# nmoehrle/mvs-texturing

Measured on AMD Instinct MI355X. Metric: faces/sec through view-selection (data-cost + MRF), higher is better.
Workload: dtype f32; 1 GPU; BASELINE config 3: displaced icosphere n=316 (1997120 faces), 200 Fibonacci-sphere views 2048x1536 RGB8, settings gmi/none/visibility-test (reference defaults); faces=1997120, views=200, nnz=88914367, sweeps=39, icm_iters=10, partition=library-hilbert-1, face_order_in=as built, msg_bits=8, max_labels=0

## Files before the change

### mvs-texturing_amd/csrc/ctx.h

```cpp
#pragma once
#include <hip/hip_runtime.h>
#include <stdint.h>
#include <string.h>
#include <algorithm>
#include <functional>
#include <stdexcept>
#include <string>
#include <vector>

#include "../../include/mvs_viewsel.h"
#include "dmath.h"

namespace mvs {

struct HipError : std::runtime_error {
    explicit HipError(const std::string& m) : std::runtime_error(m) {}
};
struct StatusError : std::runtime_error {
    mvs_status st;
    StatusError(mvs_status s, const std::string& m) : std::runtime_error(m), st(s) {}
};

#define MVS_HIP(expr)                                                                          \
    do {                                                                                       \
// ... 133 lines not shown
    mvs::DBuf<size_t> view_off;
    bool mesh_dirty = true, views_dirty = true;

    int face_order = 1;
    mvs::DBuf<float> i_verts, i_normals; mvs::DBuf<uint32_t> i_faces, f_perm, f_pos, f_tmp;
    const float* iv = nullptr; const uint32_t* ifc = nullptr; const float* inr = nullptr;
    bool mesh_ordered = false;
    bool order_pinned = false;
    const uint32_t* t_perm = nullptr; const uint32_t* t_pos = nullptr;
    mvs::DBuf<uint32_t> u_ptr, u_cnt; mvs::DBuf<uint16_t> u_view; mvs::DBuf<float> u_cost, u_q;
    bool u_valid = false, u_q_valid = false;
    mvs::DBuf<unsigned long long> fp_acc;
    mvs::HBuf<uint32_t> stage_ptr; mvs::HBuf<uint16_t> stage_view[2]; mvs::HBuf<float> stage_cost[2];

    mvs::DBuf<mvs::Node4> bvh_nodes; mvs::DBuf<float4> bvh_tris;
    mvs::DBuf<uint32_t> sort_k, sort_k2, sort_v, sort_v2; mvs::DBuf<char> sort_tmp;
    mvs::DBuf<float> lvl_box_a, lvl_box_b; mvs::DBuf<float> scene_box;
    mvs::BvhDev bvh{};
    mvs::DBuf<uint32_t> vf_ptr, vf_cursor, vf;
    mvs::DBuf<uint32_t> vperm, vpos;
    const uint32_t* tri_order = nullptr;

    mvs::DBuf<unsigned long long> pass_bits, need_bits, occl_bits, surv_bits;
    mvs::DBuf<uint32_t> pass_base;
    mvs::DBuf<uint32_t> pass_face;
    mvs::DBuf<unsigned long long> defer_bits; mvs::DBuf<uint32_t> defer_base; mvs::DBuf<uint2> defer_list; mvs::DBuf<uint32_t> rewalk_list;
    mvs::DBuf<float> pq;
    mvs::DBuf<float> pcol;
    mvs::DBuf<uint32_t> face_cnt, scan_tmp;
    mvs::DBuf<unsigned long long> counters;
    mvs::DBuf<float> max_q; mvs::DBuf<uint32_t> hist; mvs::DBuf<float> pctl;
    mvs::DBuf<uint32_t> pre_ptr; mvs::DBuf<uint16_t> pre_view; mvs::DBuf<float> pre_q; mvs::DBuf<float> pre_col;
    mvs::DBuf<uint8_t> pre_inl;
    mvs::DBuf<uint32_t> csr_ptr; mvs::DBuf<uint16_t> csr_view; mvs::DBuf<float> csr_cost; mvs::DBuf<float> csr_q;
    uint32_t csr_faces = 0, csr_views = 0; uint64_t csr_nnz = 0;
    const uint32_t* r_ptr = nullptr; const uint16_t* r_view = nullptr; const float* r_cost = nullptr;
    bool csr_q_valid = false;
    bool have_costs = false;
    mvs_settings dc_settings{}; mvs_dc_stats dc_stats{}; int dc_phase = 0;

    mvs::DBuf<unsigned long long> g_keys, g_keys2; mvs::DBuf<uint32_t> g_vals, g_vals2, g_pos, g_cnt, g_adj_ptr, g_adj, g_faces; mvs::DBuf<float> g_normals;
    uint64_t g_adj_entries = 0; bool have_adj = false;

    mvs::DBuf<uint32_t> p_label_ptr, p_comp_ptr, p_comp_faces, p_parent, p_root, p_state, p_flag, p_pos, p_roots, p_roots2, p_rlab, p_rlab2, p_adj_ptr, p_adj, p_labels;

    mvs::DBuf<uint32_t> row_adj_ptr, row_adj, row_labels; mvs::HBuf<char> row_pin;
// ... 93 lines not shown
```

### mvs-texturing_amd/csrc/dmath.h

```cpp
#pragma once
#include <stdint.h>
#include <math.h>
#include <float.h>
#include <string.h>

#if defined(__HIPCC__)
#define MVS_HD __host__ __device__ __forceinline__
#else
#define MVS_HD inline
#endif

namespace mvs {

struct V3 { float x, y, z; };
struct V2 { float x, y; };

MVS_HD V3 operator+(V3 a, V3 b) { return {a.x + b.x, a.y + b.y, a.z + b.z}; }
MVS_HD V3 operator-(V3 a, V3 b) { return {a.x - b.x, a.y - b.y, a.z - b.z}; }
MVS_HD V3 operator/(V3 a, float s) { return {a.x / s, a.y / s, a.z / s}; }
MVS_HD float dot(V3 a, V3 b) { return (a.x * b.x + a.y * b.y) + a.z * b.z; }
MVS_HD float norm(V3 a) { return sqrtf(dot(a, a)); }
MVS_HD V3 normalized(V3 a) { return a / norm(a); }
MVS_HD V3 cross(V3 a, V3 b) {
    return {a.y * b.z - a.z * b.y, a.z * b.x - a.x * b.z, a.x * b.y - a.y * b.x};
// ... 123 lines not shown
    float ext = 0.0f, mag = 0.0f;
    for (int a = 0; a < 3; ++a) {
        ext = fmaxf(ext, hi[a] - lo[a]);
        mag = fmaxf(mag, fmaxf(fabsf(lo[a]), fabsf(hi[a])));
    }
    return 1e-5f * fmaxf(ext, mag) + 1e-30f;
}

MVS_HD void tri_pad_box(V3 a, V3 e1, V3 e2, float pad, V3* lo, V3* hi) {
    const V3 b = a + e1, c = a + e2;
    lo->x = fminf(a.x, fminf(b.x, c.x)) - pad; hi->x = fmaxf(a.x, fmaxf(b.x, c.x)) + pad;
    lo->y = fminf(a.y, fminf(b.y, c.y)) - pad; hi->y = fmaxf(a.y, fmaxf(b.y, c.y)) + pad;
    lo->z = fminf(a.z, fminf(b.z, c.z)) - pad; hi->z = fmaxf(a.z, fmaxf(b.z, c.z)) + pad;
}
MVS_HD float dot_fma(V3 a, V3 b) { return __builtin_fmaf(a.z, b.z, __builtin_fmaf(a.y, b.y, a.x * b.x)); }
MVS_HD V3 cross_fma(V3 a, V3 b) {
    return V3{__builtin_fmaf(a.y, b.z, -(a.z * b.y)), __builtin_fmaf(a.z, b.x, -(a.x * b.z)), __builtin_fmaf(a.x, b.y, -(a.y * b.x))};
}
MVS_HD bool ray_tri_point_in_box(const Ray& r, float tn, float det, V3 lo, V3 hi) {
    const float t = tn / det;
    const float hx = r.o.x + t * r.d.x, hy = r.o.y + t * r.d.y, hz = r.o.z + t * r.d.z;
    return hx >= lo.x && hx <= hi.x && hy >= lo.y && hy <= hi.y && hz >= lo.z && hz <= hi.z;
}
MVS_HD bool ray_tri_boxed(const Ray& r, V3 a, V3 e1, V3 e2, V3 lo, V3 hi) {
    const V3 pv = cross_fma(r.d, e2);
    const float det = dot_fma(e1, pv);
    const V3 tv = r.o - a;
    const float un = dot_fma(tv, pv);
    const V3 qv = cross_fma(tv, e1);
    const float vn = dot_fma(r.d, qv);
    const float tn = dot_fma(e2, qv);
    const float sg = det < 0.0f ? -1.0f : 1.0f;
    const float ad = det * sg, us = un * sg, vs = vn * sg, ts = tn * sg;
    const float w = ad - (us + vs);
    const float g1 = __builtin_fmaf(-r.tmin, ad, ts), g2 = __builtin_fmaf(r.tmax, ad, -ts);
    const bool pre = (ad > 0.0f) & (fminf(fminf(fminf(fminf(us, vs), w), g1), g2) >= 0.0f);
    if (!pre) return false;
    return ray_tri_point_in_box(r, tn, det, lo, hi);
}
MVS_HD bool ray_tri(const Ray& r, V3 a, V3 e1, V3 e2) {
    V3 lo, hi;
    tri_pad_box(a, e1, e2, r.pad, &lo, &hi);
    return ray_tri_boxed(r, a, e1, e2, lo, hi);
}

MVS_HD uint8_t linear_at(const uint8_t* img, int w, int h, int chans, float x, float y, int c) {
    x = smax(0.0f, smin((float)(w - 1), x));
    y = smax(0.0f, smin((float)(h - 1), y));
    const int floor_x = (int)x, floor_y = (int)y;
    const int floor_xp1 = imin(floor_x + 1, w - 1), floor_yp1 = imin(floor_y + 1, h - 1);
    const float w1 = x - (float)floor_x, w0 = 1.0f - w1;
    const float w3 = y - (float)floor_y, w2 = 1.0f - w3;
    const int rowstride = w * chans;
    const size_t row1 = (size_t)floor_y * rowstride, row2 = (size_t)floor_yp1 * rowstride;
    const int col1 = floor_x * chans, col2 = floor_xp1 * chans;
    const float v1 = img[row1 + col1 + c], v2 = img[row1 + col2 + c];
    const float v3 = img[row2 + col1 + c], v4 = img[row2 + col2 + c];
    return (uint8_t)(((v1 * (w0 * w2) + v2 * (w1 * w2)) + v3 * (w0 * w3)) + v4 * (w1 * w3) + 0.5f);
}

// ... 261 lines not shown
```

### mvs-texturing_amd/csrc/k_bvh.hip

```cpp
#include "ctx.h"
#include <rocprim/rocprim.hpp>
#ifndef MVS_LEAF_T
#define MVS_LEAF_T 16
#endif

namespace mvs {

namespace {

constexpr uint32_t LEAF_T = MVS_LEAF_T;
constexpr int LEAF_SLOTS = 64 / (int)LEAF_T;

__device__ __forceinline__ uint32_t f2ord(float f) {
    uint32_t u = __float_as_uint(f);
    return (u & 0x80000000u) ? ~u : (u | 0x80000000u);
}
__device__ __forceinline__ float ord2f(uint32_t u) {
    return __uint_as_float((u & 0x80000000u) ? (u & 0x7FFFFFFFu) : ~u);
}

__global__ void __launch_bounds__(256) bbox_kernel(const float* __restrict__ verts, uint32_t n_verts, uint32_t* __restrict__ part ) {
    __shared__ uint32_t s_red[4][6];
    float lo[3] = {INFINITY, INFINITY, INFINITY}, hi[3] = {-INFINITY, -INFINITY, -INFINITY};
    for (uint32_t v = blockIdx.x * blockDim.x + threadIdx.x; v < n_verts; v += gridDim.x * blockDim.x)
// ... 156 lines not shown
    float lo[3], hi[3];
    for (int a = 0; a < 3; ++a) { lo[a] = ord2f(box[a]); hi[a] = ord2f(box[3 + a]); }
    return scene_pad(lo, hi);
}

constexpr uint32_t TRI_F4 = 4;
__global__ void gather_tris_kernel(const float* __restrict__ verts, const uint32_t* __restrict__ faces, const uint32_t* __restrict__ order,
                                   uint32_t n_faces, uint32_t n_slots, const uint32_t* __restrict__ scene_box, float4* __restrict__ tris) {
    const uint32_t s = blockIdx.x * blockDim.x + threadIdx.x;
    if (s >= n_slots) return;
    float4 a = {0, 0, 0, 0}, e1 = {0, 0, 0, 0}, e2 = {0, 0, 0, 0}, h = {0, 0, 0, 0};
    if (s < n_faces) {
        const uint32_t* fv = faces + 3 * (size_t)(order ? order[s] : s);
        const V3 pa = {verts[3 * (size_t)fv[0]], verts[3 * (size_t)fv[0] + 1], verts[3 * (size_t)fv[0] + 2]};
        const V3 pb = {verts[3 * (size_t)fv[1]], verts[3 * (size_t)fv[1] + 1], verts[3 * (size_t)fv[1] + 2]};
        const V3 pc = {verts[3 * (size_t)fv[2]], verts[3 * (size_t)fv[2] + 1], verts[3 * (size_t)fv[2] + 2]};
        const V3 d1 = pb - pa, d2 = pc - pa;
        V3 lo, hi;
        tri_pad_box(pa, d1, d2, pad_from_box(scene_box), &lo, &hi);
        a = {pa.x, pa.y, pa.z, lo.x}; e1 = {d1.x, d1.y, d1.z, lo.y}; e2 = {d2.x, d2.y, d2.z, lo.z}; h = {hi.x, hi.y, hi.z, 0.0f};
    }
    float4* t = tris + TRI_F4 * (size_t)s;
    t[0] = a; t[1] = e1; t[2] = e2; t[3] = h;
}
__device__ __forceinline__ bool tri_hit(const float4 A, const float4 E1, const float4 E2, const float4 H, const Ray& r) {
    return ray_tri_boxed(r, V3{A.x, A.y, A.z}, V3{E1.x, E1.y, E1.z}, V3{E2.x, E2.y, E2.z}, V3{A.w, E1.w, E2.w}, V3{H.x, H.y, H.z});
}

__global__ void build_level0_kernel(const float4* __restrict__ tris, uint32_t n_faces, uint32_t n_leaves, uint32_t n_nodes,
                                    const uint32_t* __restrict__ scene_box, Node4* __restrict__ nodes, float* __restrict__ own_box) {
    const uint32_t n = blockIdx.x * blockDim.x + threadIdx.x;
    if (n >= n_nodes) return;
    float slo[3], shi[3];
    for (int a = 0; a < 3; ++a) { slo[a] = ord2f(scene_box[a]); shi[a] = ord2f(scene_box[3 + a]); }
    const float pad = scene_pad(slo, shi);
    Node4 nd;
    float nlo[3] = {INFINITY, INFINITY, INFINITY}, nhi[3] = {-INFINITY, -INFINITY, -INFINITY};
    uint32_t nchild = 0;
    for (int c = 0; c < 4; ++c) {
        const uint32_t leaf = 4 * n + c;
        float lo[3] = {1e30f, 1e30f, 1e30f}, hi[3] = {1e30f, 1e30f, 1e30f};
        if (leaf < n_leaves) {
            nchild = c + 1;
            for (int a = 0; a < 3; ++a) { lo[a] = INFINITY; hi[a] = -INFINITY; }
            for (uint32_t t = LEAF_T * leaf; t < LEAF_T * leaf + LEAF_T && t < n_faces; ++t) {
                const float4 A = tris[TRI_F4 * (size_t)t], E1 = tris[TRI_F4 * (size_t)t + 1], E2 = tris[TRI_F4 * (size_t)t + 2];
                const float pa[3] = {A.x, A.y, A.z};
                const float pb[3] = {A.x + E1.x, A.y + E1.y, A.z + E1.z};
                const float pc[3] = {A.x + E2.x, A.y + E2.y, A.z + E2.z};
// ... 32 lines not shown
        for (int a = 0; a < 3; ++a) { nd.b[c][a] = lo[a]; nd.b[c][3 + a] = hi[a]; }
    }
    nd.nchild = nchild;
    for (int k = 0; k < 7; ++k) nd.pad_[k] = 0;
    nodes[n] = nd;
    for (int a = 0; a < 3; ++a) { own_box[6 * (size_t)n + a] = nlo[a]; own_box[6 * (size_t)n + 3 + a] = nhi[a]; }
}

__global__ void vf_count_kernel(const uint32_t* __restrict__ faces, uint32_t n_faces, uint32_t* __restrict__ deg) {
    const uint32_t i = blockIdx.x * blockDim.x + threadIdx.x;
    if (i >= 3 * n_faces) return;
    atomicAdd(&deg[faces[i]], 1u);
}
__global__ void vf_fill_kernel(const uint32_t* __restrict__ faces, uint32_t n_faces, const uint32_t* __restrict__ vf_ptr,
                               uint32_t* __restrict__ cursor, uint32_t* __restrict__ vf) {
    const uint32_t i = blockIdx.x * blockDim.x + threadIdx.x;
    if (i >= 3 * n_faces) return;
    const uint32_t v = faces[i];
    const uint32_t k = atomicAdd(&cursor[v], 1u);
    vf[vf_ptr[v] + k] = i / 3;
}

typedef float f2 __attribute__((ext_vector_type(2)));

__device__ __forceinline__ uint32_t shift_in_nonzero(uint32_t m, unsigned long long mask) {
    asm("s_cmp_lg_u64 %1, 0\n\ts_addc_u32 %0, %0, %0" : "+s"(m) : "s"(mask) : "scc");
    return m;
}
__device__ __forceinline__ unsigned long long clear_bit(unsigned long long x, uint32_t bit) {
    asm("s_bitset0_b64 %0, %1" : "+s"(x) : "s"(bit));
    return x;
}

template <int OCT, bool COUNT>
__device__ __forceinline__ void packet3_traverse(const BvhDev& bvh, const float4 (*s_ray)[2], uint8_t* s_src, const int lane, const float pad,
                                                 const V3 inv, const V3 oi, const float t0, float t1,
                                                 unsigned long long& actm , uint32_t (&cnt)[3] ) {
    constexpr bool SX = (OCT & 1) != 0, SY = (OCT & 2) != 0, SZ = (OCT & 4) != 0, GEN = OCT >= 8;
    const f2 I0 = {inv.x, inv.y}, I1 = {inv.z, inv.x}, I2 = {inv.y, inv.z};
    const f2 O0 = {-oi.x, -oi.y}, O1 = {-oi.z, -oi.x}, O2 = {-oi.y, -oi.z};
    const Node4* __restrict__ nodes = bvh.nodes;
    t1 = __builtin_amdgcn_inverse_ballot_w64(actm) ? t1 : -1.0f;
    unsigned long long hm0 = 0ull, hm1 = 0ull, hm2 = 0ull, hm3 = 0ull;
    auto fetch = [&](uint32_t h) -> Node4 {
        if (COUNT) ++cnt[0];
        return *reinterpret_cast<const Node4*>(reinterpret_cast<const char*>(nodes) + (h << 7));
    };
    auto test = [&](const Node4& nd) -> uint32_t {
        uint32_t m = 0;
#pragma unroll
        for (int c = 3; c >= 0; --c) {
            const f2 P0 = {nd.b[c][0], nd.b[c][1]}, P1 = {nd.b[c][2], nd.b[c][3]}, P2 = {nd.b[c][4], nd.b[c][5]};
            const f2 R0 = __builtin_elementwise_fma(P0, I0, O0);
            const f2 R1 = __builtin_elementwise_fma(P1, I1, O1);
            const f2 R2 = __builtin_elementwise_fma(P2, I2, O2);
            float tn, tf;
            if (GEN) {
                tn = fmaxf(t0, fminf(R0.x, R1.y)); tf = fminf(t1, fmaxf(R0.x, R1.y));
                tn = fmaxf(tn, fminf(R0.y, R2.x)); tf = fminf(tf, fmaxf(R0.y, R2.x));
                tn = fmaxf(tn, fminf(R1.x, R2.y)); tf = fminf(tf, fmaxf(R1.x, R2.y));
            } else {
                const float nx = SX ? R1.y : R0.x, fx = SX ? R0.x : R1.y;
                const float ny = SY ? R2.x : R0.y, fy = SY ? R0.y : R2.x;
                const float nz = SZ ? R2.y : R1.x, fz = SZ ? R1.x : R2.y;
                tn = fmaxf(fmaxf(fmaxf(nx, ny), nz), t0);
                tf = fminf(fminf(fminf(fx, fy), fz), t1);
            }
            const unsigned long long hb = __builtin_amdgcn_ballot_w64(tn <= tf);
            if (c == 0) hm0 = hb; else if (c == 1) hm1 = hb; else if (c == 2) hm2 = hb; else hm3 = hb;
            m = shift_in_nonzero(m, hb);
        }
        return m;
    };
    auto visit = [&](uint32_t h) -> uint32_t { const Node4 nd = fetch(h); return test(nd); };
    auto leaves = [&](uint32_t h0, uint32_t m) {
        const uint32_t leaf0 = (h0 - bvh.level_off[0]) * 4u;
        while (m != 0u) {
            const uint32_t c = (uint32_t)__builtin_ctz(m);
            m &= m - 1u;
            unsigned long long hsel = (c == 1u) ? hm1 : hm0;
            asm("" : "+s"(hsel));
            hsel = (c == 2u) ? hm2 : hsel;
            asm("" : "+s"(hsel));
            hsel = (c == 3u) ? hm3 : hsel;
            const unsigned long long cb = hsel & actm;
            if (cb != 0ull) {
                const bool cand = __builtin_amdgcn_inverse_ballot_w64(cb);
                const int n = __builtin_popcountll(cb);
                const int rank = (int)__builtin_amdgcn_mbcnt_hi((uint32_t)(cb >> 32), __builtin_amdgcn_mbcnt_lo((uint32_t)cb, 0u));
                if (cand) s_src[rank] = (uint8_t)lane;
                const float4* __restrict__ tp = bvh.tris + TRI_F4 * (size_t)((leaf0 + c) * LEAF_T + ((uint32_t)lane & (LEAF_T - 1u)));
                const float4 A = tp[0], E1 = tp[1], E2 = tp[2], H = tp[3];
                unsigned long long hitm = 0ull;
                if (COUNT) { ++cnt[1]; cnt[2] += (uint32_t)((n + LEAF_SLOTS - 1) / LEAF_SLOTS); }
                for (int base = 0; base < n; base += LEAF_SLOTS) {
                    const int q = base + lane / (int)LEAF_T;
                    const int sl = (int)s_src[q];
                    const float4 r0 = s_ray[sl][0], r1 = s_ray[sl][1];
                    Ray rr; rr.o = V3{r0.x, r0.y, r0.z}; rr.tmin = r0.w; rr.d = V3{r1.x, r1.y, r1.z}; rr.tmax = r1.w; rr.pad = pad;
                    const bool h = tri_hit(A, E1, E2, H, rr) && q < n;
                    const unsigned long long hb = __builtin_amdgcn_ballot_w64(h);
                    if (hb != 0ull) {
                        const bool mine = cand && rank >= base && rank < base + LEAF_SLOTS &&
                                          ((hb >> ((int)LEAF_T * (rank - base))) & ((1ull << LEAF_T) - 1ull)) != 0ull;
                        hitm |= __builtin_amdgcn_ballot_w64(mine);
                    }
                }
                if (hitm != 0ull) {
                    actm &= ~hitm;
                    t1 = __builtin_amdgcn_inverse_ballot_w64(actm) ? t1 : -1.0f;
                    if (actm == 0ull) m = 0u;
                }
            }
        }
    };
    const uint32_t top = (uint32_t)bvh.top;
    uint32_t m = visit(1u);
    if (top == 0u) { leaves(1u, m); return; }
    unsigned long long masks = (unsigned long long)m << (4u * top);
    uint32_t level = top, h = 1u;
    if (masks == 0ull) return;
    const char* __restrict__ nbase = reinterpret_cast<const char*>(nodes);
    (void)nbase;
#ifndef MVS_RAY_PREFETCH
    do {
        const uint32_t idx = (uint32_t)__builtin_ctzll(masks);
        masks = clear_bit(masks, idx);
        const uint32_t lv = idx >> 2;
        const uint32_t ch = ((h >> (2u * (lv - level))) << 2) | (idx & 3u);
        m = visit(ch);
        if (lv != 1u) { masks |= (unsigned long long)m << (4u * (lv - 1u)); h = ch; level = lv - 1u; }
        else { h = ch >> 2; level = 1u; leaves(ch, m); masks = (actm == 0ull) ? 0ull : masks; }
    } while (masks != 0ull);
#else
    uint32_t idx = (uint32_t)__builtin_ctzll(masks);
    masks = clear_bit(masks, idx);
    uint32_t lv = idx >> 2, ch = ((h >> (2u * (lv - level))) << 2) | (idx & 3u);
    Node4 nd = fetch(ch);
    for (;;) {
        m = test(nd);
        if (lv != 1u) {
            masks |= (unsigned long long)m << (4u * (lv - 1u)); h = ch; level = lv - 1u;
            if (masks == 0ull) break;
            idx = (uint32_t)__builtin_ctzll(masks); masks = clear_bit(masks, idx);
            lv = idx >> 2; ch = ((h >> (2u * (lv - level))) << 2) | (idx & 3u);
            nd = fetch(ch);
        } else {
            const uint32_t leaf_node = ch;
            h = ch >> 2; level = 1u;
            const bool more = masks != 0ull;
            if (more) {
                idx = (uint32_t)__builtin_ctzll(masks); masks = clear_bit(masks, idx);
                lv = idx >> 2; ch = ((h >> (2u * (lv - level))) << 2) | (idx & 3u);
                nd = fetch(ch);
            }
            leaves(leaf_node, m);
            if (!more || actm == 0ull) break;
        }
    }
#endif
}

template <bool XCD, bool COUNT>
__global__ void __launch_bounds__(256, 8) __attribute__((amdgpu_num_sgpr(80))) ray_packet3_kernel(const BvhDev bvh, const float* __restrict__ verts ,
                                                          const ViewParams* __restrict__ views, const unsigned long long* __restrict__ need,
                                                          unsigned long long* __restrict__ occl, uint32_t vwords, uint32_t n_verts, uint32_t n_views,
                                                          const uint32_t* __restrict__ scene_box, unsigned long long* __restrict__ counters) {
    __shared__ float4 s_ray[4][64][2];
    __shared__ uint8_t s_src[4][80];
    uint32_t vblk = blockIdx.x;
    if (XCD && (gridDim.x & 7u) == 0u) vblk = (blockIdx.x & 7u) * (gridDim.x >> 3) + (blockIdx.x >> 3);
    const uint64_t wave = ((uint64_t)vblk * blockDim.x + threadIdx.x) >> 6;
    const int lane = threadIdx.x & 63, wv = threadIdx.x >> 6;
    if (wave >= (uint64_t)vwords * n_views) return;
    const uint32_t j = (uint32_t)(wave / vwords), vw = (uint32_t)(wave % vwords);
    const unsigned long long word = need[(size_t)j * vwords + vw];
    if (word == 0ull) return;
    const uint32_t s = vw * 64 + lane;
    const bool active = ((word >> lane) & 1ull) && s < n_verts;
    const uint32_t v = s < n_verts ? s : 0;
    const ViewParams& vp = views[j];
    const V3 o = {verts[3 * (size_t)v], verts[3 * (size_t)v + 1], verts[3 * (size_t)v + 2]};
    const float pad = pad_from_box(scene_box);
    const Ray r = make_ray(o, V3{vp.pos[0], vp.pos[1], vp.pos[2]}, pad);
    s_ray[wv][lane][0] = make_float4(r.o.x, r.o.y, r.o.z, r.tmin);
    s_ray[wv][lane][1] = make_float4(r.d.x, r.d.y, r.d.z, r.tmax);
    s_src[wv][lane] = (uint8_t)lane; if (lane < 16) s_src[wv][64 + lane] = (uint8_t)lane;
    const V3 inv = {1.0f / r.d.x, 1.0f / r.d.y, 1.0f / r.d.z};
    const V3 oi = {r.o.x * inv.x, r.o.y * inv.y, r.o.z * inv.z};
    const float t0 = r.tmin * 0.999f, t1 = r.tmax * 1.001f;
    const unsigned long long actm = __builtin_amdgcn_ballot_w64(active);
    unsigned long long live = actm;
    const float big = 1e30f;
    const unsigned long long okm = __builtin_amdgcn_ballot_w64(fabsf(inv.x) < big && fabsf(inv.y) < big && fabsf(inv.z) < big) & actm;
    const unsigned long long nxm = __builtin_amdgcn_ballot_w64(inv.x < 0.0f) & actm, nym = __builtin_amdgcn_ballot_w64(inv.y < 0.0f) & actm,
                             nzm = __builtin_amdgcn_ballot_w64(inv.z < 0.0f) & actm;
    int oct = 8;
    if (okm == actm && (nxm == 0ull || nxm == actm) && (nym == 0ull || nym == actm) && (nzm == 0ull || nzm == actm))
        oct = (nxm ? 1 : 0) | (nym ? 2 : 0) | (nzm ? 4 : 0);
    if (counters && lane == 0) { atomicAdd(&counters[10], 1ull); if (oct == 8) atomicAdd(&counters[11], 1ull); }
    uint32_t cnt[3] = {0u, 0u, 0u};
#define MVS_P3(O) packet3_traverse<O, COUNT>(bvh, s_ray[wv], s_src[wv], lane, pad, inv, oi, t0, t1, live, cnt)
    switch (oct) {
        case 0: MVS_P3(0); break; case 1: MVS_P3(1); break; case 2: MVS_P3(2); break; case 3: MVS_P3(3); break;
        case 4: MVS_P3(4); break; case 5: MVS_P3(5); break; case 6: MVS_P3(6); break; case 7: MVS_P3(7); break;
        default: MVS_P3(8); break;
    }
#undef MVS_P3
    if (lane == 0) occl[(size_t)j * vwords + vw] = actm & ~live;
    if (COUNT && lane == 0) { atomicAdd(&counters[8], (unsigned long long)cnt[0]); atomicAdd(&counters[9], (unsigned long long)cnt[1]); atomicAdd(&counters[13], (unsigned long long)cnt[2]); }
}

}

void build_vertex_faces(mvs_ctx* ctx, const uint32_t* d_faces, uint32_t F, uint32_t NV) {
    hipStream_t s = ctx->stream;
    ctx->vf_ptr.ensure((size_t)NV + 1); ctx->vf_cursor.ensure((size_t)NV + 1); ctx->vf.ensure(3 * (size_t)F + 1);
    MVS_HIP(hipMemsetAsync(ctx->vf_cursor.p, 0, ((size_t)NV + 1) * sizeof(uint32_t), s));
    if (F) { hipLaunchKernelGGL(vf_count_kernel, dim3((3 * F + 255) / 256), dim3(256), 0, s, d_faces, F, ctx->vf_cursor.p); MVS_LAUNCH_CHECK(); }
    exclusive_scan_u32(ctx, ctx->vf_cursor.p, ctx->vf_ptr.p, (size_t)NV + 1, nullptr);
    MVS_HIP(hipMemsetAsync(ctx->vf_cursor.p, 0, ((size_t)NV + 1) * sizeof(uint32_t), s));
    if (F) { hipLaunchKernelGGL(vf_fill_kernel, dim3((3 * F + 255) / 256), dim3(256), 0, s, d_faces, F, ctx->vf_ptr.p, ctx->vf_cursor.p, ctx->vf.p); MVS_LAUNCH_CHECK(); }
}

namespace {
// ... 127 lines not shown
    }
    b.top = L; b.n_leaves = n_leaves;
    for (int l = 0; l <= L; ++l) {
        uint64_t p4 = 1; for (int k = 0; k < L - l; ++k) p4 *= 4;
        if (p4 + b.level_cnt[l] > 0x01FFFFFFull) throw HipError("BVH too large");
        b.level_off[l] = (uint32_t)p4;
    }
    const uint32_t off = b.level_off[0] + b.level_cnt[0];
    ctx->bvh_nodes.ensure(std::max<uint32_t>(off, 256u));
    ctx->lvl_box_a.ensure(6 * (size_t)b.level_cnt[0]); ctx->lvl_box_b.ensure(6 * (size_t)std::max<uint32_t>(b.level_cnt[L > 0 ? 1 : 0], 1u));
    hipLaunchKernelGGL(build_level0_kernel, dim3((b.level_cnt[0] + 127) / 128), dim3(128), 0, s, ctx->bvh_tris.p, F, n_leaves, b.level_cnt[0], box, ctx->bvh_nodes.p + b.level_off[0], ctx->lvl_box_a.p);
    MVS_LAUNCH_CHECK();
    float* cur = ctx->lvl_box_a.p; float* nxt = ctx->lvl_box_b.p;
    for (int l = 1; l <= L; ++l) {
        hipLaunchKernelGGL(build_level_kernel, dim3((b.level_cnt[l] + 127) / 128), dim3(128), 0, s, cur, b.level_cnt[l - 1], b.level_cnt[l], ctx->bvh_nodes.p + b.level_off[l], nxt);
        MVS_LAUNCH_CHECK();
        std::swap(cur, nxt);
    }
    b.nodes = ctx->bvh_nodes.p; b.tris = ctx->bvh_tris.p;
    ctx->bvh = b;
    build_vertex_faces(ctx, ctx->ifc, F, NV);
}

void trace_rays(mvs_ctx* ctx) {
    const uint32_t vwords = (ctx->n_verts + 63) / 64;
    const uint64_t waves = (uint64_t)vwords * ctx->n_views;
    uint64_t blocks = (waves + 3) / 4;
    blocks = (blocks + 7) & ~7ull;
    if (blocks > 0x7FFFFFFFull) throw HipError("ray grid too large");
    unsigned long long* counters = (ctx->stats || ctx->count_rays) ? ctx->counters.p : nullptr;
#define RAY_ARGS dim3((unsigned)blocks), dim3(256), 0, ctx->stream, ctx->bvh, ctx->iv, ctx->d_views.p, ctx->need_bits.p, ctx->occl_bits.p, \
                 vwords, ctx->n_verts, ctx->n_views, (const uint32_t*)ctx->scene_box.p, counters
    if (ctx->count_rays) { if (ctx->ray_xcd) hipLaunchKernelGGL((ray_packet3_kernel<true, true>), RAY_ARGS); else hipLaunchKernelGGL((ray_packet3_kernel<false, true>), RAY_ARGS); }
    else { if (ctx->ray_xcd) hipLaunchKernelGGL((ray_packet3_kernel<true, false>), RAY_ARGS); else hipLaunchKernelGGL((ray_packet3_kernel<false, false>), RAY_ARGS); }
#undef RAY_ARGS
    MVS_LAUNCH_CHECK();
}

}
```

### mvs-texturing_amd/csrc/k_dc.hip

```cpp
#include "ctx.h"

namespace mvs {

void prepare_views(mvs_ctx* ctx, bool need_gmi, const size_t* d_gmi_off, const size_t* d_mask_off);
void build_scene_order(mvs_ctx* ctx);
bool scene_order_commit(mvs_ctx* ctx);
void build_bvh(mvs_ctx* ctx);
void trace_rays(mvs_ctx* ctx);

namespace {

constexpr int VIEW_CHUNK = 32;
constexpr uint32_t HIST_BINS = 10000;

enum { C_BACK = 0, C_ANGLE = 1, C_OUTSIDE = 2, C_OCCL = 3, C_ZEROQ = 4, C_SURV = 5, C_RAYS = 6, C_PASS = 7, C_RNODES = 8, C_RTRIS = 9, C_REWALK = 12 };

__device__ __forceinline__ V3 ld3(const float* __restrict__ p, size_t i) { return {p[3 * i], p[3 * i + 1], p[3 * i + 2]}; }

__device__ __forceinline__ uint32_t wave_sum(uint32_t v) {
    for (int o = 32; o > 0; o >>= 1) v += __shfl_xor(v, o, 64);
    return v;
}
template <int N>
__device__ __forceinline__ void block_count_add(const uint32_t (&c)[N], unsigned long long* __restrict__ counters, const int (&slot)[N]) {
    __shared__ uint32_t acc[N];
    if (threadIdx.x < N) acc[threadIdx.x] = 0;
    __syncthreads();
#pragma unroll
    for (int k = 0; k < N; ++k) { const uint32_t w = wave_sum(c[k]); if ((threadIdx.x & 63) == 0 && w) atomicAdd(&acc[k], w); }
    __syncthreads();
    if (threadIdx.x < N && acc[threadIdx.x]) atomicAdd(&counters[slot[threadIdx.x]], (unsigned long long)acc[threadIdx.x]);
// ... 17 lines not shown
        const uint32_t n_chunks = (n_views + VIEW_CHUNK - 1) / VIEW_CHUNK, per = (n_chunks + gridDim.y - 1) / gridDim.y;
        const uint32_t c_begin = blockIdx.y * per, c_end = min(c_begin + per, n_chunks);
        for (uint32_t chunk = c_begin, j0 = c_begin * VIEW_CHUNK; chunk < c_end; j0 += VIEW_CHUNK, ++chunk) {
            const uint32_t j1 = min(j0 + VIEW_CHUNK, n_views);
            uint32_t mine = 0;
            for (uint32_t j = j0; j < j1; ++j) {
                const ViewParams& vw = views[j];
                const int reason = act ? cull_pair_prefiltered(vw, v1, v2, v3, nrm, centre, cos_limit) : -1;
                if (STATS) { cnt[0] += reason == 1; cnt[1] += reason == 2; cnt[2] += reason == 3; cnt[3] += reason == 0; }
                const unsigned long long b = __ballot(reason == 0);
                if (lane == 0) pass[(size_t)j * fwords + (lf >> 6)] = b;
                mine |= (reason == 0 ? 1u : 0u) << (j - j0);
            }
            if (pass_face) pass_face[(size_t)chunk * ((size_t)fwords * 64u) + lf] = mine;
        }
    }
    if (STATS) { const int slot[4] = {C_BACK, C_ANGLE, C_OUTSIDE, C_PASS}; block_count_add<4>(cnt, counters, slot); }
}

template <bool STATS>
__global__ void __launch_bounds__(256) need_kernel(const uint32_t* __restrict__ vf_ptr, const uint32_t* __restrict__ vf, uint32_t n_verts, uint32_t n_views,
                                                   uint32_t fb, uint32_t nf, uint32_t fwords, uint32_t vwords,
                                                   const uint32_t* __restrict__ pass_face ,
                                                   unsigned long long* __restrict__ need, unsigned long long* __restrict__ counters) {
    const uint32_t v = blockIdx.x * 256 + threadIdx.x;
    if ((v >> 6) >= vwords) return;
    const bool act = v < n_verts;
    const uint32_t vid = act ? v : 0;
    const uint32_t p0 = act ? vf_ptr[vid] : 0, p1 = act ? vf_ptr[vid + 1] : 0;
    const uint32_t j0 = blockIdx.y * VIEW_CHUNK, j1 = min(j0 + VIEW_CHUNK, n_views);
    const int lane = threadIdx.x & 63;
    uint32_t acc = 0;
    for (uint32_t pb = p0; pb < p1; pb += 4) {
        uint32_t lf[4], w[4];
#pragma unroll
        for (int t = 0; t < 4; ++t) lf[t] = (pb + t < p1) ? vf[pb + t] - fb : 0xFFFFFFFFu;
#pragma unroll
        for (int t = 0; t < 4; ++t) w[t] = (lf[t] < nf) ? pass_face[(size_t)blockIdx.y * ((size_t)fwords * 64u) + lf[t]] : 0u;
        acc |= (w[0] | w[1]) | (w[2] | w[3]);
    }
    uint32_t n_rays = 0;
    for (uint32_t j = j0; j < j1; ++j) {
        const unsigned long long b = __ballot((acc >> (j - j0)) & 1u);
        if (lane == 0) { need[(size_t)j * vwords + (v >> 6)] = b; n_rays += __popcll(b); }
    }
    if (STATS && lane == 0 && n_rays) atomicAdd(&counters[C_RAYS], (unsigned long long)n_rays);
}

__global__ void popc_kernel(const unsigned long long* __restrict__ words, uint32_t* __restrict__ cnt, size_t n) {
    const size_t i = (size_t)blockIdx.x * blockDim.x + threadIdx.x;
    if (i < n) cnt[i] = (uint32_t)__popcll(words[i]);
}

template <int DATA_TERM, bool OUTLIER, bool VISTEST, bool STATS, bool WORDS>
__global__ void __launch_bounds__(256, WORDS ? 6 : 1) info_kernel(const float* __restrict__ verts, const uint32_t* __restrict__ faces, const ViewParams* __restrict__ views,
                                                   uint32_t n_views, uint32_t fb, uint32_t nf, uint32_t fwords, uint32_t vwords,
                                                   const unsigned long long* __restrict__ pass, const unsigned long long* __restrict__ occl,
                                                   const uint32_t* __restrict__ pass_base, float* __restrict__ pq, float* __restrict__ pcol,
                                                   unsigned long long* __restrict__ surv, unsigned long long* __restrict__ counters,
                                                   float defer_area ,
                                                   unsigned long long* __restrict__ defer_bits, int cert_shift) {
    static_assert(!WORDS || (DATA_TERM == 1 && !OUTLIER), "the word walk sums gradient magnitudes only");
    __shared__ double s_q255[WORDS ? 1 : 256];
    if (!WORDS) {
        s_q255[threadIdx.x] = (double)threadIdx.x / 255.0;
        __syncthreads();
    }
// ... 700 lines not shown
        struct Swap { mvs_ctx* c; hipStream_t main; ~Swap() { c->stream = main; } } swap{ctx, s};
        ctx->stream = ctx->aux_stream;
        { Prof pr(ctx, "dc_prep"); upload_views_and_prepare(ctx, gmi); }
        MVS_HIP(hipEventRecord(ctx->ev_join, ctx->aux_stream));
        ctx->stream = s;
        MVS_HIP(hipStreamWaitEvent(s, ctx->ev_join, 0));
    }

    const size_t pw = (size_t)V * fwords;
    ctx->pass_bits.ensure(pw + 1); ctx->surv_bits.ensure(pw + 1); ctx->pass_base.ensure(pw + 2);
    const dim3 fgrid((nf + 255) / 256, (V + VIEW_CHUNK - 1) / VIEW_CHUNK);
    uint32_t* pass_face = nullptr;
    if (vis) { ctx->pass_face.ensure((size_t)fgrid.y * fwords * 64u + 1); pass_face = ctx->pass_face.p; }
    Prof pr_cull(ctx, "dc_cull");
    const dim3 cgrid(fgrid.x, std::max(1u, std::min<unsigned>(fgrid.y, (4096u + fgrid.x - 1) / fgrid.x)));
    if (ctx->stats)
        hipLaunchKernelGGL(cull_kernel<true>, cgrid, dim3(256), 0, s, ctx->iv, ctx->ifc, ctx->inr, ctx->d_views.p, V, fb, nf, fwords,
                           ctx->cos_limit, ctx->pass_bits.p, pass_face, ctx->counters.p);
    else
        hipLaunchKernelGGL(cull_kernel<false>, cgrid, dim3(256), 0, s, ctx->iv, ctx->ifc, ctx->inr, ctx->d_views.p, V, fb, nf, fwords,
                           ctx->cos_limit, ctx->pass_bits.p, pass_face, ctx->counters.p);
    MVS_LAUNCH_CHECK();
    pr_cull.end();
    if (vis) {
        const size_t vw = (size_t)V * vwords;
        ctx->need_bits.ensure(vw + 1); ctx->occl_bits.ensure(vw + 1);
        MVS_HIP(hipMemsetAsync(ctx->occl_bits.p, 0, vw * sizeof(unsigned long long), s));
        const dim3 vgrid((ctx->n_verts + 255) / 256, (V + VIEW_CHUNK - 1) / VIEW_CHUNK);
        Prof pr_need(ctx, "dc_need");
        if (ctx->stats)
            hipLaunchKernelGGL(need_kernel<true>, vgrid, dim3(256), 0, s, ctx->vf_ptr.p, ctx->vf.p, ctx->n_verts, V, fb, nf, fwords, vwords,
                               pass_face, ctx->need_bits.p, ctx->counters.p);
        else
            hipLaunchKernelGGL(need_kernel<false>, vgrid, dim3(256), 0, s, ctx->vf_ptr.p, ctx->vf.p, ctx->n_verts, V, fb, nf, fwords, vwords,
                               pass_face, ctx->need_bits.p, ctx->counters.p);
        MVS_LAUNCH_CHECK();
        pr_need.end();
        Prof pr_rays(ctx, "dc_rays");
        trace_rays(ctx);
        pr_rays.end();
    }
    Prof pr_rank(ctx, "dc_rank_scan");
    hipLaunchKernelGGL(popc_kernel, dim3((unsigned)((pw + 255) / 256)), dim3(256), 0, s, ctx->pass_bits.p, ctx->pass_base.p, pw);
    MVS_LAUNCH_CHECK();
    ctx->max_q.ensure(4);
    uint32_t* d_total = (uint32_t*)(ctx->max_q.p + 2);
    if ((uint64_t)nf * V >= 0xFFFFFFF0ull && sum_u32(ctx, ctx->pass_base.p, pw) >= 0xFFFFFFF0ull)
        throw StatusError(MVS_ERR_UNSUPPORTED, "more than 2^32 (face, view) pairs pass the culls in one context: evaluate the faces in ranges (mvs_scene_set_face_range)");
    exclusive_scan_u32(ctx, ctx->pass_base.p, ctx->pass_base.p, pw, d_total);
    pr_rank.end();
    const uint32_t n_pass = read_word(ctx, d_total);
    if (scene_order_commit(ctx)) return true;
    ctx->pq.ensure((size_t)n_pass + 1);
    if (outl) ctx->pcol.ensure(3 * ((size_t)n_pass + 1));

    Prof pr_info(ctx, "dc_face_info");
    const bool defer = (gmi || outl) && ctx->info_wave_area > 0;
    ctx->dc_stats_deferred = 0;
    const bool words = defer && ctx->info_words && gmi && !outl;
    const float defer_area = defer ? (float)(words ? std::max(ctx->info_wave_area, ctx->info_wave_area_words) : ctx->info_wave_area) : INFINITY;
    unsigned long long* defer_bits = nullptr;
    if (defer) { ctx->defer_bits.ensure(pw + 1); defer_bits = ctx->defer_bits.p; }
#define LAUNCH_INFO(DT, OL, VT, WD)                                                                                          \
    do { if (ctx->stats) LAUNCH_INFO2(DT, OL, VT, true, WD); else LAUNCH_INFO2(DT, OL, VT, false, WD); } while (0)
#define LAUNCH_INFO2(DT, OL, VT, ST, WD)                                                                                     \
    hipLaunchKernelGGL((info_kernel<DT, OL, VT, ST, WD>), fgrid, dim3(256), 0, s, ctx->iv, ctx->ifc, ctx->d_views.p, V, fb, nf, \
                       fwords, vwords, ctx->pass_bits.p, ctx->occl_bits.p, ctx->pass_base.p, ctx->pq.p, ctx->pcol.p,         \
                       ctx->surv_bits.p, ctx->counters.p, defer_area, defer_bits, ctx->info_cert_shift)
    if (gmi) { if (outl) { if (vis) LAUNCH_INFO(1, true, true, false); else LAUNCH_INFO(1, true, false, false); }
               else if (words) { if (vis) LAUNCH_INFO(1, false, true, true); else LAUNCH_INFO(1, false, false, true); }
               else      { if (vis) LAUNCH_INFO(1, false, true, false); else LAUNCH_INFO(1, false, false, false); } }
    else     { if (outl) { if (vis) LAUNCH_INFO(0, true, true, false); else LAUNCH_INFO(0, true, false, false); }
               else      { if (vis) LAUNCH_INFO(0, false, true, false); else LAUNCH_INFO(0, false, false, false); } }
#undef LAUNCH_INFO
#undef LAUNCH_INFO2
// ... 303 lines not shown
```

Before: 76.48 million faces/s.

## Compact nonzero ray packets into a list and stage leaf triangles through LDS

The need kernel now also flags which (view, vertex-word) packets have any rays. A scan plus a small kernel compacts these into a packet list, so the ray kernel launches only waves that have work instead of exiting empty waves early. Ray tracing is moved after the pass scan so the packet count can be read back together with the pass total in a single readback. Leaf triangles are loaded coalesced, one float4 per lane, into padded LDS, with the next leaf prefetched. The bounding-box data is fetched only after the Möller-Trumbore pre-test passes. The change adds a scan, an extra kernel, LDS use and the removal of the unused prefetch variant.

```diff
diff --git a/mvs-texturing_amd/csrc/ctx.h b/mvs-texturing_amd/csrc/ctx.h
--- a/mvs-texturing_amd/csrc/ctx.h
+++ b/mvs-texturing_amd/csrc/ctx.h
@@ -179,6 +179,7 @@
     const uint32_t* tri_order = nullptr;
 
     mvs::DBuf<unsigned long long> pass_bits, need_bits, occl_bits, surv_bits;
+    mvs::DBuf<uint32_t> ray_base, ray_packet;
     mvs::DBuf<uint32_t> pass_base;
     mvs::DBuf<uint32_t> pass_face;
     mvs::DBuf<unsigned long long> defer_bits; mvs::DBuf<uint32_t> defer_base; mvs::DBuf<uint2> defer_list; mvs::DBuf<uint32_t> rewalk_list;
diff --git a/mvs-texturing_amd/csrc/dmath.h b/mvs-texturing_amd/csrc/dmath.h
--- a/mvs-texturing_amd/csrc/dmath.h
+++ b/mvs-texturing_amd/csrc/dmath.h
@@ -169,7 +169,7 @@
     const float hx = r.o.x + t * r.d.x, hy = r.o.y + t * r.d.y, hz = r.o.z + t * r.d.z;
     return hx >= lo.x && hx <= hi.x && hy >= lo.y && hy <= hi.y && hz >= lo.z && hz <= hi.z;
 }
-MVS_HD bool ray_tri_boxed(const Ray& r, V3 a, V3 e1, V3 e2, V3 lo, V3 hi) {
+MVS_HD bool ray_tri_pre(const Ray& r, V3 a, V3 e1, V3 e2, float* tn_out, float* det_out) {
     const V3 pv = cross_fma(r.d, e2);
     const float det = dot_fma(e1, pv);
     const V3 tv = r.o - a;
@@ -182,7 +182,12 @@
     const float w = ad - (us + vs);
     const float g1 = __builtin_fmaf(-r.tmin, ad, ts), g2 = __builtin_fmaf(r.tmax, ad, -ts);
     const bool pre = (ad > 0.0f) & (fminf(fminf(fminf(fminf(us, vs), w), g1), g2) >= 0.0f);
-    if (!pre) return false;
+    *tn_out = tn; *det_out = det;
+    return pre;
+}
+MVS_HD bool ray_tri_boxed(const Ray& r, V3 a, V3 e1, V3 e2, V3 lo, V3 hi) {
+    float tn, det;
+    if (!ray_tri_pre(r, a, e1, e2, &tn, &det)) return false;
     return ray_tri_point_in_box(r, tn, det, lo, hi);
 }
 MVS_HD bool ray_tri(const Ray& r, V3 a, V3 e1, V3 e2) {
diff --git a/mvs-texturing_amd/csrc/k_bvh.hip b/mvs-texturing_amd/csrc/k_bvh.hip
--- a/mvs-texturing_amd/csrc/k_bvh.hip
+++ b/mvs-texturing_amd/csrc/k_bvh.hip
@@ -202,9 +202,6 @@
     }
     float4* t = tris + TRI_F4 * (size_t)s;
     t[0] = a; t[1] = e1; t[2] = e2; t[3] = h;
-}
-__device__ __forceinline__ bool tri_hit(const float4 A, const float4 E1, const float4 E2, const float4 H, const Ray& r) {
-    return ray_tri_boxed(r, V3{A.x, A.y, A.z}, V3{E1.x, E1.y, E1.z}, V3{E2.x, E2.y, E2.z}, V3{A.w, E1.w, E2.w}, V3{H.x, H.y, H.z});
 }
 
 __global__ void build_level0_kernel(const float4* __restrict__ tris, uint32_t n_faces, uint32_t n_leaves, uint32_t n_nodes,
@@ -283,6 +280,8 @@
 }
 
 typedef float f2 __attribute__((ext_vector_type(2)));
+constexpr int TRI_LDS_F4 = (int)TRI_F4 + 1;
+static_assert(TRI_F4 * LEAF_T == 64, "a leaf is staged as one float4 per lane");
 
 __device__ __forceinline__ uint32_t shift_in_nonzero(uint32_t m, unsigned long long mask) {
     asm("s_cmp_lg_u64 %1, 0\n\ts_addc_u32 %0, %0, %0" : "+s"(m) : "s"(mask) : "scc");
@@ -294,7 +293,7 @@
 }
 
 template <int OCT, bool COUNT>
-__device__ __forceinline__ void packet3_traverse(const BvhDev& bvh, const float4 (*s_ray)[2], uint8_t* s_src, const int lane, const float pad,
+__device__ __forceinline__ void packet3_traverse(const BvhDev& bvh, const float4 (*s_ray)[2], uint8_t* s_src, float4* s_tri, const int lane, const float pad,
                                                  const V3 inv, const V3 oi, const float t0, float t1,
                                                  unsigned long long& actm , uint32_t (&cnt)[3] ) {
     constexpr bool SX = (OCT & 1) != 0, SY = (OCT & 2) != 0, SZ = (OCT & 4) != 0, GEN = OCT >= 8;
@@ -336,6 +335,10 @@
     auto visit = [&](uint32_t h) -> uint32_t { const Node4 nd = fetch(h); return test(nd); };
     auto leaves = [&](uint32_t h0, uint32_t m) {
         const uint32_t leaf0 = (h0 - bvh.level_off[0]) * 4u;
+        const float4* __restrict__ tl = bvh.tris + (uint32_t)lane;
+        const int wr = (lane >> 2) * TRI_LDS_F4 + (lane & 3), rd = (lane & (int)(LEAF_T - 1u)) * TRI_LDS_F4;
+        bool ahead = false;
+        float4 stage = {0.0f, 0.0f, 0.0f, 0.0f};
         while (m != 0u) {
             const uint32_t c = (uint32_t)__builtin_ctz(m);
             m &= m - 1u;
@@ -350,8 +353,12 @@
                 const int n = __builtin_popcountll(cb);
                 const int rank = (int)__builtin_amdgcn_mbcnt_hi((uint32_t)(cb >> 32), __builtin_amdgcn_mbcnt_lo((uint32_t)cb, 0u));
                 if (cand) s_src[rank] = (uint8_t)lane;
-                const float4* __restrict__ tp = bvh.tris + TRI_F4 * (size_t)((leaf0 + c) * LEAF_T + ((uint32_t)lane & (LEAF_T - 1u)));
-                const float4 A = tp[0], E1 = tp[1], E2 = tp[2], H = tp[3];
+                if (!ahead) stage = tl[(size_t)(leaf0 + c) * (TRI_F4 * LEAF_T)];
+                s_tri[wr] = stage;
+                const float4 A4 = s_tri[rd], E14 = s_tri[rd + 1], E24 = s_tri[rd + 2];
+                const V3 A = {A4.x, A4.y, A4.z}, E1 = {E14.x, E14.y, E14.z}, E2 = {E24.x, E24.y, E24.z};
+                ahead = m != 0u;
+                if (ahead) stage = tl[(size_t)(leaf0 + (uint32_t)__builtin_ctz(m)) * (TRI_F4 * LEAF_T)];
                 unsigned long long hitm = 0ull;
                 if (COUNT) { ++cnt[1]; cnt[2] += (uint32_t)((n + LEAF_SLOTS - 1) / LEAF_SLOTS); }
                 for (int base = 0; base < n; base += LEAF_SLOTS) {
@@ -359,7 +366,12 @@
                     const int sl = (int)s_src[q];
                     const float4 r0 = s_ray[sl][0], r1 = s_ray[sl][1];
                     Ray rr; rr.o = V3{r0.x, r0.y, r0.z}; rr.tmin = r0.w; rr.d = V3{r1.x, r1.y, r1.z}; rr.tmax = r1.w; rr.pad = pad;
-                    const bool h = tri_hit(A, E1, E2, H, rr) && q < n;
+                    float tn, det;
+                    bool h = false;
+                    if (ray_tri_pre(rr, A, E1, E2, &tn, &det)) {
+                        const float4 H = s_tri[rd + 3];
+                        h = ray_tri_point_in_box(rr, tn, det, V3{s_tri[rd].w, s_tri[rd + 1].w, s_tri[rd + 2].w}, V3{H.x, H.y, H.z}) && q < n;
+                    }
                     const unsigned long long hb = __builtin_amdgcn_ballot_w64(h);
                     if (hb != 0ull) {
                         const bool mine = cand && rank >= base && rank < base + LEAF_SLOTS &&
@@ -372,7 +384,7 @@
                     t1 = __builtin_amdgcn_inverse_ballot_w64(actm) ? t1 : -1.0f;
                     if (actm == 0ull) m = 0u;
                 }
-            }
+            } else ahead = false;
         }
     };
     const uint32_t top = (uint32_t)bvh.top;
@@ -381,9 +393,6 @@
     unsigned long long masks = (unsigned long long)m << (4u * top);
     uint32_t level = top, h = 1u;
     if (masks == 0ull) return;
-    const char* __restrict__ nbase = reinterpret_cast<const char*>(nodes);
-    (void)nbase;
-#ifndef MVS_RAY_PREFETCH
     do {
         const uint32_t idx = (uint32_t)__builtin_ctzll(masks);
         masks = clear_bit(masks, idx);
@@ -393,48 +402,25 @@
         if (lv != 1u) { masks |= (unsigned long long)m << (4u * (lv - 1u)); h = ch; level = lv - 1u; }
         else { h = ch >> 2; level = 1u; leaves(ch, m); masks = (actm == 0ull) ? 0ull : masks; }
     } while (masks != 0ull);
-#else
-    uint32_t idx = (uint32_t)__builtin_ctzll(masks);
-    masks = clear_bit(masks, idx);
-    uint32_t lv = idx >> 2, ch = ((h >> (2u * (lv - level))) << 2) | (idx & 3u);
-    Node4 nd = fetch(ch);
-    for (;;) {
-        m = test(nd);
-        if (lv != 1u) {
-            masks |= (unsigned long long)m << (4u * (lv - 1u)); h = ch; level = lv - 1u;
-            if (masks == 0ull) break;
-            idx = (uint32_t)__builtin_ctzll(masks); masks = clear_bit(masks, idx);
-            lv = idx >> 2; ch = ((h >> (2u * (lv - level))) << 2) | (idx & 3u);
-            nd = fetch(ch);
-        } else {
-            const uint32_t leaf_node = ch;
-            h = ch >> 2; level = 1u;
-            const bool more = masks != 0ull;
-            if (more) {
-                idx = (uint32_t)__builtin_ctzll(masks); masks = clear_bit(masks, idx);
-                lv = idx >> 2; ch = ((h >> (2u * (lv - level))) << 2) | (idx & 3u);
-                nd = fetch(ch);
-            }
-            leaves(leaf_node, m);
-            if (!more || actm == 0ull) break;
-        }
-    }
-#endif
 }
 
 template <bool XCD, bool COUNT>
 __global__ void __launch_bounds__(256, 8) __attribute__((amdgpu_num_sgpr(80))) ray_packet3_kernel(const BvhDev bvh, const float* __restrict__ verts ,
                                                           const ViewParams* __restrict__ views, const unsigned long long* __restrict__ need,
-                                                          unsigned long long* __restrict__ occl, uint32_t vwords, uint32_t n_verts, uint32_t n_views,
+                                                          unsigned long long* __restrict__ occl, const uint32_t* __restrict__ packet ,
+                                                          uint64_t n_waves, uint32_t vwords, uint32_t n_verts,
                                                           const uint32_t* __restrict__ scene_box, unsigned long long* __restrict__ counters) {
     __shared__ float4 s_ray[4][64][2];
     __shared__ uint8_t s_src[4][80];
+    __shared__ float4 s_tri[4][LEAF_T * TRI_LDS_F4];
     uint32_t vblk = blockIdx.x;
     if (XCD && (gridDim.x & 7u) == 0u) vblk = (blockIdx.x & 7u) * (gridDim.x >> 3) + (blockIdx.x >> 3);
-    const uint64_t wave = ((uint64_t)vblk * blockDim.x + threadIdx.x) >> 6;
-    const int lane = threadIdx.x & 63, wv = threadIdx.x >> 6;
-    if (wave >= (uint64_t)vwords * n_views) return;
-    const uint32_t j = (uint32_t)(wave / vwords), vw = (uint32_t)(wave % vwords);
+    const int lane = threadIdx.x & 63, wv = __builtin_amdgcn_readfirstlane((int)(threadIdx.x >> 6));
+    const uint64_t wave = (uint64_t)vblk * (blockDim.x >> 6) + (uint32_t)wv;
+    if (wave >= n_waves) return;
+    uint32_t j, vw;
+    if (packet) { const uint32_t i = packet[wave]; j = i / vwords; vw = i - j * vwords; }
+    else { j = (uint32_t)(wave / vwords); vw = (uint32_t)(wave % vwords); }
     const unsigned long long word = need[(size_t)j * vwords + vw];
     if (word == 0ull) return;
     const uint32_t s = vw * 64 + lane;
@@ -461,7 +447,7 @@
         oct = (nxm ? 1 : 0) | (nym ? 2 : 0) | (nzm ? 4 : 0);
     if (counters && lane == 0) { atomicAdd(&counters[10], 1ull); if (oct == 8) atomicAdd(&counters[11], 1ull); }
     uint32_t cnt[3] = {0u, 0u, 0u};
-#define MVS_P3(O) packet3_traverse<O, COUNT>(bvh, s_ray[wv], s_src[wv], lane, pad, inv, oi, t0, t1, live, cnt)
+#define MVS_P3(O) packet3_traverse<O, COUNT>(bvh, s_ray[wv], s_src[wv], s_tri[wv], lane, pad, inv, oi, t0, t1, live, cnt)
     switch (oct) {
         case 0: MVS_P3(0); break; case 1: MVS_P3(1); break; case 2: MVS_P3(2); break; case 3: MVS_P3(3); break;
         case 4: MVS_P3(4); break; case 5: MVS_P3(5); break; case 6: MVS_P3(6); break; case 7: MVS_P3(7); break;
@@ -635,15 +621,34 @@
     build_vertex_faces(ctx, ctx->ifc, F, NV);
 }
 
-void trace_rays(mvs_ctx* ctx) {
+namespace {
+__global__ void __launch_bounds__(256) ray_packet_list_kernel(const unsigned long long* __restrict__ need, const uint32_t* __restrict__ base, uint32_t n,
+                                                              uint32_t* __restrict__ packet) {
+    const uint32_t i = blockIdx.x * 256u + threadIdx.x;
+    if (i < n && need[i] != 0ull) packet[base[i]] = i;
+}
+}
+void list_ray_packets(mvs_ctx* ctx, uint32_t* d_count) {
+    const uint64_t n = (uint64_t)((ctx->n_verts + 63) / 64) * ctx->n_views;
+    if (n > 0xFFFFFFFFull) throw HipError("ray packet list: more need words than 32 bits count");
+    exclusive_scan_u32(ctx, ctx->ray_base.p, ctx->ray_base.p, (size_t)n, d_count);
+    if (n == 0) return;
+    hipLaunchKernelGGL(ray_packet_list_kernel, dim3((unsigned)((n + 255) / 256)), dim3(256), 0, ctx->stream, (const unsigned long long*)ctx->need_bits.p,
+                       (const uint32_t*)ctx->ray_base.p, (uint32_t)n, ctx->ray_packet.p);
+    MVS_LAUNCH_CHECK();
+}
+
+void trace_rays(mvs_ctx* ctx, bool from_list, uint32_t n_packets) {
     const uint32_t vwords = (ctx->n_verts + 63) / 64;
-    const uint64_t waves = (uint64_t)vwords * ctx->n_views;
+    const uint64_t waves = from_list ? (uint64_t)n_packets : (uint64_t)vwords * ctx->n_views;
+    if (waves == 0) return;
     uint64_t blocks = (waves + 3) / 4;
     blocks = (blocks + 7) & ~7ull;
     if (blocks > 0x7FFFFFFFull) throw HipError("ray grid too large");
     unsigned long long* counters = (ctx->stats || ctx->count_rays) ? ctx->counters.p : nullptr;
+    const uint32_t* packet = from_list ? ctx->ray_packet.p : nullptr;
 #define RAY_ARGS dim3((unsigned)blocks), dim3(256), 0, ctx->stream, ctx->bvh, ctx->iv, ctx->d_views.p, ctx->need_bits.p, ctx->occl_bits.p, \
-                 vwords, ctx->n_verts, ctx->n_views, (const uint32_t*)ctx->scene_box.p, counters
+                 packet, waves, vwords, ctx->n_verts, (const uint32_t*)ctx->scene_box.p, counters
     if (ctx->count_rays) { if (ctx->ray_xcd) hipLaunchKernelGGL((ray_packet3_kernel<true, true>), RAY_ARGS); else hipLaunchKernelGGL((ray_packet3_kernel<false, true>), RAY_ARGS); }
     else { if (ctx->ray_xcd) hipLaunchKernelGGL((ray_packet3_kernel<true, false>), RAY_ARGS); else hipLaunchKernelGGL((ray_packet3_kernel<false, false>), RAY_ARGS); }
 #undef RAY_ARGS
diff --git a/mvs-texturing_amd/csrc/k_dc.hip b/mvs-texturing_amd/csrc/k_dc.hip
--- a/mvs-texturing_amd/csrc/k_dc.hip
+++ b/mvs-texturing_amd/csrc/k_dc.hip
@@ -6,7 +6,8 @@
 void build_scene_order(mvs_ctx* ctx);
 bool scene_order_commit(mvs_ctx* ctx);
 void build_bvh(mvs_ctx* ctx);
-void trace_rays(mvs_ctx* ctx);
+void list_ray_packets(mvs_ctx* ctx, uint32_t* d_count);
+void trace_rays(mvs_ctx* ctx, bool from_list, uint32_t n_packets);
 
 namespace {
 
@@ -70,7 +71,8 @@
 __global__ void __launch_bounds__(256) need_kernel(const uint32_t* __restrict__ vf_ptr, const uint32_t* __restrict__ vf, uint32_t n_verts, uint32_t n_views,
                                                    uint32_t fb, uint32_t nf, uint32_t fwords, uint32_t vwords,
                                                    const uint32_t* __restrict__ pass_face ,
-                                                   unsigned long long* __restrict__ need, unsigned long long* __restrict__ counters) {
+                                                   unsigned long long* __restrict__ need, uint32_t* __restrict__ live ,
+                                                   unsigned long long* __restrict__ counters) {
     const uint32_t v = blockIdx.x * 256 + threadIdx.x;
     if ((v >> 6) >= vwords) return;
     const bool act = v < n_verts;
@@ -90,7 +92,7 @@
     uint32_t n_rays = 0;
     for (uint32_t j = j0; j < j1; ++j) {
         const unsigned long long b = __ballot((acc >> (j - j0)) & 1u);
-        if (lane == 0) { need[(size_t)j * vwords + (v >> 6)] = b; n_rays += __popcll(b); }
+        if (lane == 0) { need[(size_t)j * vwords + (v >> 6)] = b; if (live) live[(size_t)j * vwords + (v >> 6)] = b != 0ull; n_rays += __popcll(b); }
     }
     if (STATS && lane == 0 && n_rays) atomicAdd(&counters[C_RAYS], (unsigned long long)n_rays);
 }
@@ -837,35 +839,44 @@
                            ctx->cos_limit, ctx->pass_bits.p, pass_face, ctx->counters.p);
     MVS_LAUNCH_CHECK();
     pr_cull.end();
+    ctx->max_q.ensure(4);
+    uint32_t* d_total = (uint32_t*)(ctx->max_q.p + 2);
+    bool packet_list = false;
     if (vis) {
         const size_t vw = (size_t)V * vwords;
         ctx->need_bits.ensure(vw + 1); ctx->occl_bits.ensure(vw + 1);
         MVS_HIP(hipMemsetAsync(ctx->occl_bits.p, 0, vw * sizeof(unsigned long long), s));
+        packet_list = vw <= 0xFFFFFFFFull;
+        if (packet_list) { ctx->ray_base.ensure(vw + 2); ctx->ray_packet.ensure(vw + 1); }
+        uint32_t* live = packet_list ? ctx->ray_base.p : nullptr;
         const dim3 vgrid((ctx->n_verts + 255) / 256, (V + VIEW_CHUNK - 1) / VIEW_CHUNK);
         Prof pr_need(ctx, "dc_need");
         if (ctx->stats)
             hipLaunchKernelGGL(need_kernel<true>, vgrid, dim3(256), 0, s, ctx->vf_ptr.p, ctx->vf.p, ctx->n_verts, V, fb, nf, fwords, vwords,
-                               pass_face, ctx->need_bits.p, ctx->counters.p);
+                               pass_face, ctx->need_bits.p, live, ctx->counters.p);
         else
             hipLaunchKernelGGL(need_kernel<false>, vgrid, dim3(256), 0, s, ctx->vf_ptr.p, ctx->vf.p, ctx->n_verts, V, fb, nf, fwords, vwords,
-                               pass_face, ctx->need_bits.p, ctx->counters.p);
+                               pass_face, ctx->need_bits.p, live, ctx->counters.p);
         MVS_LAUNCH_CHECK();
+        if (packet_list) list_ray_packets(ctx, d_total + 1);
         pr_need.end();
-        Prof pr_rays(ctx, "dc_rays");
-        trace_rays(ctx);
-        pr_rays.end();
     }
     Prof pr_rank(ctx, "dc_rank_scan");
     hipLaunchKernelGGL(popc_kernel, dim3((unsigned)((pw + 255) / 256)), dim3(256), 0, s, ctx->pass_bits.p, ctx->pass_base.p, pw);
     MVS_LAUNCH_CHECK();
-    ctx->max_q.ensure(4);
-    uint32_t* d_total = (uint32_t*)(ctx->max_q.p + 2);
     if ((uint64_t)nf * V >= 0xFFFFFFF0ull && sum_u32(ctx, ctx->pass_base.p, pw) >= 0xFFFFFFF0ull)
         throw StatusError(MVS_ERR_UNSUPPORTED, "more than 2^32 (face, view) pairs pass the culls in one context: evaluate the faces in ranges (mvs_scene_set_face_range)");
     exclusive_scan_u32(ctx, ctx->pass_base.p, ctx->pass_base.p, pw, d_total);
     pr_rank.end();
-    const uint32_t n_pass = read_word(ctx, d_total);
+    uint32_t h_total[2] = {0u, 0u};
+    read_words(ctx, d_total, h_total, packet_list ? 2u : 1u);
+    const uint32_t n_pass = h_total[0];
     if (scene_order_commit(ctx)) return true;
+    if (vis) {
+        Prof pr_rays(ctx, "dc_rays");
+        trace_rays(ctx, packet_list, h_total[1]);
+        pr_rays.end();
+    }
     ctx->pq.ensure((size_t)n_pass + 1);
     if (outl) ctx->pcol.ensure(3 * ((size_t)n_pass + 1));
 
```

Result: slower. 73.53 million faces/s (-3.9%).
